# Luka140/paig_reproduction

Hardware: AMD Instinct MI355X
Metric: video-seqs/sec (train step) spring_color B=100 @ 1/2/4/8 MI355X (higher is better)
Workload: dtype fp32; 1 GPU; spring_color PhysicsNet train step (get_batch gather+fwd+loss+bwd+allreduce+RMSprop), B=100/rank, 32x32x3, seq_len 50 (4 in / 6 pred / 40 extrap); global_batch=100, seq_len=50, parallelism=dp1, conv_math=split, split_graph=False, optimizer_in_graph=True, byte_targets=True, dataset_seqs=800

## Files before the change

### paig_reproduction_amd/csrc/conv_split.hip

```cpp
#include "split_common.h"

#ifndef PAIG_FWD_AUXP
#define PAIG_FWD_AUXP 1
#endif

namespace {


constexpr bool sfwd_sla(bool UPS, int PM, int H, int W, int ups_bytes, int lo_bytes) {
  return UPS && PM == 0 && H * W >= 4096 && ups_bytes <= lo_bytes;
}
constexpr int sfwd_lds(int CIN, int H, int W, int KS, bool UPS, int PM, int tpxm, int ntb) {
  const int CC = rup(CIN, 8) / 8, PS = CC % 2 == 0 ? CC + 1 : CC;
  const int NS = ceil_div(KS * KS * CC, 4);
  const int FPT = H * W <= tpxm ? tpxm / (H * W) : 1;
  const int RT = H * W <= tpxm ? H : rows_fit(H, W, tpxm);
  const int TWPX = W + 2 * (KS / 2);
  const int RP = W == 8 ? to_mod16(TWPX * PS, 8) : TWPX * PS;
  const int img = FPT * (RT + KS - 1) * RP * 8, wimg = NS * ntb * 64 * 8;
  const int ups = UPS ? up_window_floats(CIN, FPT, RT, W) * 4 : 0;
  return (img + wimg) * 2 * (PM == 2 ? 1 : 2) + (sfwd_sla(UPS, PM, H, W, ups, img * 2) ? 0 : ups);
}
constexpr int sfwd_vgprs(int CIN, int H, int W, int KS, bool UPS, int tpxm, int ntb) {
  const int CC = rup(CIN, 8) / 8, NS = ceil_div(KS * KS * CC, 4);
  const int FPT = H * W <= tpxm ? tpxm / (H * W) : 1;
  const int RT = H * W <= tpxm ? H : rows_fit(H, W, tpxm);
  const int MW = ceil_div(ceil_div(FPT * RT * W, 16), 4);
  const int NL = UPS ? 1 : ceil_div(FPT * (RT + KS - 1) * (W % 2 == 0 ? W / 2 : W) * CC, 256);
  return MW * ntb * 4 + NL * 30 + ntb * 8 + NS + MW * 8 + 40;
}
#ifndef PAIG_FWD_UPS_TP
#define PAIG_FWD_UPS_TP 256
#endif
#ifndef PAIG_FWD_TP32
#define PAIG_FWD_TP32 256
#endif
constexpr int sfwd_pick(int CIN, int COUT, int H, int W, int KS, bool UPS, int PM) {
  const int base = UPS && H * W < 4096 && PAIG_FWD_UPS_TP < 256   ? PAIG_FWD_UPS_TP
                   : !UPS && H * W == 1024 && PAIG_FWD_TP32 < 256 ? PAIG_FWD_TP32
                                                                  : (W == 8 ? 128 : 256);
  const int NT = ceil_div(COUT, 16);
  for (int pass = UPS && !(PM == 0 && H * W >= 4096) ? 1 : 0; pass < 3; ++pass)
    for (int nb = 1; nb <= NT; ++nb) {
      if (NT % nb != 0 || NT / nb > 4) continue;
      for (int tp = base; tp >= (pass == 1 ? base / 2 : 64); tp /= 2)
        if (sfwd_lds(CIN, H, W, KS, UPS, PM, tp, NT / nb) <= (pass == 0 ? LDS_MAX / 2 : LDS_MAX) &&
            sfwd_vgprs(CIN, H, W, KS, UPS, tp, NT / nb) <= 264 && (pass > 0 || tp >= base / 2))
          return tp * 256 + nb;
    }
  return 0;
}

template <int CIN, int COUT, int H, int W, int KS, bool UPS, int PM>
struct SFwdCfg {
  static constexpr int KK = KS * KS, PADL = KS / 2;
  static constexpr int NIMG = PM == 2 ? 1 : 2;
  static constexpr int CINP = rup(CIN, 8), CC = CINP / 8;
  static constexpr int KC = KK * CC, NS = ceil_div(KC, 4);
  static constexpr int GEO = sfwd_pick(CIN, COUT, H, W, KS, UPS, PM);
  static_assert(GEO > 0, "no forward tile geometry fits the LDS");
  static constexpr int NB = GEO % 256;
  static constexpr int NT = ceil_div(COUT, 16) / NB;
  static constexpr int TPXM = GEO / 256;
  static constexpr int FPT = H * W <= TPXM ? TPXM / (H * W) : 1;
  static constexpr int RT = H * W <= TPXM ? H : rows_fit(H, W, TPXM);
  static constexpr int TPXV = FPT * RT * W;
  static constexpr int NMT = ceil_div(TPXV, 16);
  static constexpr int MW = ceil_div(NMT, 4);
  static constexpr int ROWS = RT + KS - 1;
  static constexpr int TWPX = W + 2 * PADL;
  static constexpr int PS = CC % 2 == 0 ? CC + 1 : CC;
  static constexpr int RP = W == 8 ? to_mod16(TWPX * PS, 8) : TWPX * PS;
  static constexpr int IMG = FPT * ROWS * RP * 8;
  static constexpr int WIMG = NS * NT * 64 * 8;
  static constexpr int SLB = UPS ? up_window_floats(CIN, FPT, RT, W) * 4 : 0;
  static constexpr bool SLA = sfwd_sla(UPS, PM, H, W, SLB, IMG * 2);
  static constexpr int LDS = (IMG + WIMG) * 2 * NIMG + (SLA ? 0 : SLB);
  static constexpr int UPX = W % 2 == 0 ? 2 : 1;
  static constexpr int W2 = W / UPX;
  static constexpr int NI = FPT * ROWS * W2 * CC;
  static constexpr int NL = (NI + 255) / 256;
  static constexpr bool VEC4 = W % 4 == 0;
  static_assert(H % RT == 0, "RT divides H");
  static constexpr int PO = W / 16;
  static constexpr bool POOLOK = !UPS && VEC4 && W % 16 == 0 && PO >= 1 && MW % 2 == 0 && NMT == 4 * MW &&
                                 TPXV % (2 * W) == 0 && RT % 2 == 0;
};

__device__ __forceinline__ float pool4(float a, float b, float c, float d) {
  float m = a;
  if (b > m || b != b) m = b;
  if (c > m || c != c) m = c;
  if (d > m || d != d) m = d;
  return m;
}

__device__ __forceinline__ unsigned char pool_code(float a, float b, float c, float d) {
  float m = a;
  int k = 0;
  if (b > m || b != b) { m = b; k = 1; }
  if (c > m || c != c) { m = c; k = 2; }
  if (d > m || d != d) { m = d; k = 3; }
  return (unsigned char)((a > 0.f ? 1 : 0) | (b > 0.f ? 2 : 0) | (c > 0.f ? 4 : 0) | (d > 0.f ? 8 : 0) | (k << 4));
}

template <int MW, int PO, bool POOL>
__device__ __forceinline__ int fwd_mtile(int wv, int mt) {
  if constexpr (POOL) {
    constexpr int HM = MW / 2;
    const int u = wv * HM + mt % HM;
    return ((u / PO) * 2 + mt / HM) * PO + u % PO;
  } else {
    return wv * MW + mt;
  }
}

template <int CIN, int COUT, int H, int W, int KS, bool DG, bool UPS, int PM, bool POOL = false, bool UPT = false,
          bool PF = false>
__device__ __forceinline__ void conv_fwd_split_body(FView in, FViewW out, FView aux, const float* __restrict__ w,
                                                    const float* __restrict__ bias, int F, int flags, int ntiles, XMax xm,
                                                    const s16x8* __restrict__ wp, PoolOut pout, int bx, int gx) {
  using C = SFwdCfg<CIN, COUT, H, W, KS, UPS, PM>;
  static_assert(!PF || (DG && !UPS && !POOL && !UPT && C::UPX == 2 && H % 2 == 0 && CIN % 8 == 0),
                "pool fold: dgrad staging units of one window's pixel pair");
  static_assert(!UPT || (DG && !UPS && !POOL && C::FPT == 1 && C::RT % 2 == 0 && C::VEC4 && W % 2 == 0),
                "transposed-upsample epilogue: dgrad tiles of whole row pairs");
  constexpr int KK = C::KK, CC = C::CC, KC = C::KC, NS = C::NS, NT = C::NT, MW = C::MW;
  constexpr int RT = C::RT, FPT = C::FPT, ROWS = C::ROWS, PS = C::PS, RP = C::RP;
  constexpr int NI = C::NI, NL = C::NL, PADL = C::PADL, W2 = C::W2;
  constexpr long long PLANE = UPS ? (long long)(H / 2) * (W / 2) : (long long)H * W;
  constexpr long long HW = (long long)H * W;
  extern __shared__ __attribute__((aligned(16))) short lds16[];
  short* Xh = lds16;
  short* Xl = Xh + (C::NIMG == 2 ? C::IMG : 0);
  short* Wh = lds16 + C::NIMG * C::IMG;
  short* Wl = Wh + (C::NIMG == 2 ? C::WIMG : 0);
  const int tid = threadIdx.x, lane = tid & 63, wv = tid >> 6, g = lane >> 4;
  constexpr int NRB = H / RT;
  const int co0 = blockIdx.y * NT * 16;
  float rmax = 0.f;
  __shared__ float smax[4];

  auto wval = [&](int idx, int j) {
    const int ln = idx & 63, snt = idx >> 6, nt = snt % NT, s = snt / NT;
    const int kc = 4 * s + (ln >> 4), co = co0 + nt * 16 + (ln & 15);
    float v = 0.f;
    if (kc < KC && co < COUT) {
      const int tap = kc / CC, ci = (kc % CC) * 8 + j;
      if (ci < CIN) v = DG ? w[(ci * COUT + co) * KK + (KK - 1 - tap)] : w[(co * CIN + ci) * KK + tap];
    }
    return v;
  };
  int ewn[NT];
#pragma unroll
  for (int nt = 0; nt < NT; ++nt) ewn[nt] = 0;
  __shared__ int sew[PM == 0 ? NT * 16 : 1];
  auto zero_halo = [&]() {
    if (PADL > 0) {
      for (int i = tid; i < FPT * ROWS * 2 * PADL * CC; i += 256) {
        const int cc = i % CC, hc = (i / CC) % (2 * PADL), r = i / (CC * 2 * PADL);
        const int xc = hc < PADL ? hc : W + hc;
        const int o = (r * RP + xc * PS + cc) * 8;
        *reinterpret_cast<s16x8*>(Xh + o) = s16x8{0, 0, 0, 0, 0, 0, 0, 0};
        if (PM != 2) *reinterpret_cast<s16x8*>(Xl + o) = s16x8{0, 0, 0, 0, 0, 0, 0, 0};
      }
    }
  };
  zero_halo();
  int pbase[MW];
#pragma unroll
  for (int mt = 0; mt < MW; ++mt) {
    int pix = fwd_mtile<MW, C::PO, POOL>(wv, mt) * 16 + (lane & 15);
    if (pix >= C::TPXV) pix = 0;
    const int fi = pix / (RT * W), rem = pix % (RT * W);
    pbase[mt] = (fi * ROWS + rem / W) * RP + (rem % W) * PS;
  }
  int soff[NS];
#pragma unroll
  for (int s = 0; s < NS; ++s) {
    int kc = 4 * s + g;
    if (kc >= KC) kc = 0;
    const int tap = kc / CC, cc = kc % CC;
    soff[s] = (tap / KS) * RP + (tap % KS) * PS + cc;
  }

  using UP = UpStage<UPS ? CIN : 1, H, W, FPT, RT>;
  float* Sl = reinterpret_cast<float*>(C::SLA ? Xl : lds16 + C::NIMG * (C::IMG + C::WIMG));
  constexpr int UPX = C::UPX;
  auto split_px = [&](int i, const float2* v, float sc, s16x8& h0, s16x8& l0, s16x8& h1, s16x8& l1) {
    const int xp = UPX * (i % W2), r = (i / W2) % ROWS, cc = (i / (W2 * ROWS)) % CC, fi = i / (W2 * ROWS * CC);
    if constexpr (PM == 0) {
      pf32x2 sv[8];
#pragma unroll
      for (int c = 0; c < 8; ++c) sv[c] = pf32x2{v[c].x, v[c].y} * sc;
      u32x4 a0, b0, a1, b1;
#pragma unroll
      for (int k = 0; k < 4; ++k) {
        { const HiLo q_ = split_pk(sv[2 * k].x, sv[2 * k + 1].x); a0[k] = q_.h; b0[k] = q_.l; }
        { const HiLo q_ = split_pk(sv[2 * k].y, sv[2 * k + 1].y); a1[k] = q_.h; b1[k] = q_.l; }
      }
      h0 = __builtin_bit_cast(s16x8, a0);
      l0 = __builtin_bit_cast(s16x8, b0);
      h1 = __builtin_bit_cast(s16x8, a1);
      l1 = __builtin_bit_cast(s16x8, b1);
    }
    return ((fi * ROWS + r) * RP + (xp + PADL) * PS + cc) * 8;
  };
  auto put_px = [&](int i, const float2* v, float sc) {
    const int xp = UPX * (i % W2), r = (i / W2) % ROWS, cc = (i / (W2 * ROWS)) % CC, fi = i / (W2 * ROWS * CC);
    const int o = ((fi * ROWS + r) * RP + (xp + PADL) * PS + cc) * 8;
    s16x8 h0, l0, h1, l1;
    if constexpr (PM == 0) {
      pf32x2 sv[8];
#pragma unroll
      for (int c = 0; c < 8; ++c) sv[c] = pf32x2{v[c].x, v[c].y} * sc;
      u32x4 a0, b0, a1, b1;
#pragma unroll
      for (int k = 0; k < 4; ++k) {
        { const HiLo q_ = split_pk(sv[2 * k].x, sv[2 * k + 1].x); a0[k] = q_.h; b0[k] = q_.l; }
        { const HiLo q_ = split_pk(sv[2 * k].y, sv[2 * k + 1].y); a1[k] = q_.h; b1[k] = q_.l; }
      }
      h0 = __builtin_bit_cast(s16x8, a0);
      l0 = __builtin_bit_cast(s16x8, b0);
      h1 = __builtin_bit_cast(s16x8, a1);
      l1 = __builtin_bit_cast(s16x8, b1);
    } else {
#pragma unroll
      for (int c = 0; c < 8; ++c) {
        short h, lo;
        split<PM>(v[c].x, h, lo, rmax);
        h0[c] = h;
        l0[c] = lo;
        split<PM>(v[c].y, h, lo, rmax);
        h1[c] = h;
        l1[c] = lo;
      }
    }
    *reinterpret_cast<s16x8*>(Xh + o) = h0;
    if (PM != 2) *reinterpret_cast<s16x8*>(Xl + o) = l0;
    if constexpr (UPX == 2) {
      *reinterpret_cast<s16x8*>(Xh + o + PS * 8) = h1;
      if (PM != 2) *reinterpret_cast<s16x8*>(Xl + o + PS * 8) = l1;
    }
  };
  float2 pre[UPS ? 1 : NL][8];
  float dpv[PF ? NL : 1][8];
  uint2 pcv[PF ? NL : 1];
  UP up;
  constexpr bool SCL = PM == 0, DYN = PM == 0 && PAIG_SCALE_MODE < 2;
  float tsc = 1.f, tinv[NT], xrun = 0.f;
#pragma unroll
  for (int nt = 0; nt < NT; ++nt) tinv[nt] = 1.f;
  auto tile_scale = [&]() {
    const float m = fmaxf(fmaxf(smax[0], smax[1]), fmaxf(smax[2], smax[3]));
    xrun = fmaxf(xrun, m);
    const int e = f16_scale_exp(m);
    tsc = __builtin_amdgcn_ldexpf(1.f, e);
#pragma unroll
    for (int nt = 0; nt < NT; ++nt) tinv[nt] = __builtin_amdgcn_ldexpf(1.f, -(e + ewn[nt]));
  };
  auto issue = [&](int t) {
    const int f0 = (t / NRB) * FPT, y0 = (t % NRB) * RT;
    if constexpr (UPS) {
      up.issue(in, F, f0, y0, tid);
    } else {
      const float* fb = in.frame(f0);
#pragma unroll
      for (int l = 0; l < NL; ++l) {
        const int i = tid + l * 256;
        const int xp = UPX * (i % W2), r = (i / W2) % ROWS, cc = (i / (W2 * ROWS)) % CC, fi = i / (W2 * ROWS * CC);
        const int gy = y0 + r - PADL;
        const bool ok = i < NI && f0 + fi < F && gy >= 0 && gy < H;
        const int off = fi * (int)in.fs + cc * 8 * (int)PLANE + gy * W + xp;
        static_assert(8 * PLANE <= 8 * 4096, "paig_zero_planes covers the unit");
        const float* base = ok ? fb + off : paig_zero_planes;
#pragma unroll
        for (int c = 0; c < 8; ++c) {
          const float* q = CIN % 8 == 0 || cc * 8 + c < CIN ? base + c * (int)PLANE : paig_zeros;
          pre[l][c] = UPX == 2 ? *reinterpret_cast<const float2*>(q) : make_float2(*q, 0.f);
        }
        if constexpr (PF) {
          constexpr int HP = H / 2, WP = W / 2;
          const int pw = (gy >> 1) * WP + (xp >> 1);
          const float* pb = ok ? pout.frame(f0) + fi * (int)pout.fs + cc * 8 * (HP * WP) + pw : paig_zero_planes;
#pragma unroll
          for (int c = 0; c < 8; ++c) dpv[l][c] = pb[c * (HP * WP)];
          const unsigned char* cb = ok ? pout.code + (long long)(f0 + fi) * pout.code_fs + ((long long)cc * HP * WP + pw) * 8
                                       : reinterpret_cast<const unsigned char*>(paig_zeros);
          pcv[l] = *reinterpret_cast<const uint2*>(cb);
        }
      }
    }
  };
  auto fold = [&](int t) {
    if constexpr (PF) {
      const int y0 = (t % NRB) * RT;
#pragma unroll
      for (int l = 0; l < NL; ++l) {
        const int i = tid + l * 256;
        const int r = (i / W2) % ROWS;
        const int pr = ((y0 + r - PADL) & 1) * 2;
#pragma unroll
        for (int c = 0; c < 8; ++c) {
          const unsigned b = ((c < 4 ? pcv[l].x : pcv[l].y) >> (8 * (c & 3))) & 255u;
          const int am = (int)(b >> 4) & 3;
          const float vx = pre[l][c].x + (am == pr ? dpv[l][c] : 0.f);
          const float vy = pre[l][c].y + (am == pr + 1 ? dpv[l][c] : 0.f);
          pre[l][c].x = (b >> pr) & 1u ? vx : 0.f;
          pre[l][c].y = (b >> (pr + 1)) & 1u ? vy : 0.f;
        }
      }
    }
  };
  auto commit = [&](int t) {
    if constexpr (DYN) tile_scale();
    if constexpr (UPT) zero_halo();
    if constexpr (UPS) {
      const int f0 = (t / NRB) * FPT, y0 = (t % NRB) * RT;
      up.commit(Sl, tid);
      __syncthreads();
      if constexpr (C::SLA) {
        static_assert(W % 4 == 0 && UPX == 2, "SLA: 4-pixel items");
        constexpr int W4 = W / 4, NIT = ceil_div(NI / 2, 256);
        s16x8 lk[NIT][4];
        int lo_off[NIT][2];
#pragma unroll
        for (int it = 0; it < NIT; ++it) {
          const int i = tid + it * 256;
          lo_off[it][0] = -1;
          if ((NI / 2) % 256 != 0 && i >= NI / 2) break;
          const int q = i % W4, r = (i / W4) % ROWS, cc = (i / (W4 * ROWS)) % CC, fi = i / (W4 * ROWS * CC);
          const int gy = y0 + r - PADL;
          const bool ok = f0 + fi < F && gy >= 0 && gy < H;
          f32x4 o[8];
#pragma unroll
          for (int c = 0; c < 8; ++c)
            o[c] = (ok && cc * 8 + c < CIN) ? UP::row4(Sl, fi, cc * 8 + c, gy, y0, q) : f32x4{0.f, 0.f, 0.f, 0.f};
          const int ia = ((fi * CC + cc) * ROWS + r) * W2 + 2 * q;
#pragma unroll
          for (int u = 0; u < 2; ++u) {
            float2 v[8];
#pragma unroll
            for (int c = 0; c < 8; ++c) v[c] = make_float2(o[c][2 * u], o[c][2 * u + 1]);
            s16x8 h0, h1;
            const int off = split_px(ia + u, v, tsc, h0, lk[it][2 * u], h1, lk[it][2 * u + 1]);
            *reinterpret_cast<s16x8*>(Xh + off) = h0;
            *reinterpret_cast<s16x8*>(Xh + off + PS * 8) = h1;
            lo_off[it][u] = off;
          }
        }
        __syncthreads();
        for (int i = tid; i < FPT * ROWS * 2 * PADL * CC; i += 256) {
          const int cc = i % CC, hc = (i / CC) % (2 * PADL), r = i / (CC * 2 * PADL);
          const int xc = hc < PADL ? hc : W + hc;
          *reinterpret_cast<s16x8*>(Xl + (r * RP + xc * PS + cc) * 8) = s16x8{0, 0, 0, 0, 0, 0, 0, 0};
        }
#pragma unroll
        for (int it = 0; it < NIT; ++it) {
          if (lo_off[it][0] < 0) break;
#pragma unroll
          for (int u = 0; u < 2; ++u) {
            *reinterpret_cast<s16x8*>(Xl + lo_off[it][u]) = lk[it][2 * u];
            *reinterpret_cast<s16x8*>(Xl + lo_off[it][u] + PS * 8) = lk[it][2 * u + 1];
          }
        }
      } else if constexpr (W % 4 == 0) {
        constexpr int W4 = W / 4;
#pragma unroll 1
        for (int i = tid; i < NI / 2; i += 256) {
          const int q = i % W4, r = (i / W4) % ROWS, cc = (i / (W4 * ROWS)) % CC, fi = i / (W4 * ROWS * CC);
          const int gy = y0 + r - PADL;
          const bool ok = f0 + fi < F && gy >= 0 && gy < H;
          f32x4 o[8];
#pragma unroll
          for (int c = 0; c < 8; ++c)
            o[c] = (ok && cc * 8 + c < CIN) ? UP::row4(Sl, fi, cc * 8 + c, gy, y0, q) : f32x4{0.f, 0.f, 0.f, 0.f};
          const int ia = ((fi * CC + cc) * ROWS + r) * W2 + 2 * q;
          float2 v[8];
#pragma unroll
          for (int c = 0; c < 8; ++c) v[c] = make_float2(o[c][0], o[c][1]);
          put_px(ia, v, tsc);
#pragma unroll
          for (int c = 0; c < 8; ++c) v[c] = make_float2(o[c][2], o[c][3]);
          put_px(ia + 1, v, tsc);
        }
      } else {
#pragma unroll 1
        for (int i = tid; i < NI; i += 256) {
          const int xp = UPX * (i % W2), r = (i / W2) % ROWS, cc = (i / (W2 * ROWS)) % CC, fi = i / (W2 * ROWS * CC);
          const int gy = y0 + r - PADL;
          const bool ok = f0 + fi < F && gy >= 0 && gy < H;
          float2 v[8];
#pragma unroll
          for (int c = 0; c < 8; ++c)
            v[c] = (ok && cc * 8 + c < CIN)
                       ? make_float2(UP::px1(Sl, fi, cc * 8 + c, gy, y0, xp),
                                     UPX == 2 ? UP::px1(Sl, fi, cc * 8 + c, gy, y0, xp + 1) : 0.f)
                       : make_float2(0.f, 0.f);
          put_px(i, v, tsc);
        }
      }
    } else {
#pragma unroll
      for (int l = 0; l < NL; ++l) {
        const int i = tid + l * 256;
        if (NI % 256 != 0 && i >= NI) break;
        put_px(i, pre[l], tsc);
      }
    }
  };

  auto tile_max = [&]() {
    float m = 0.f;
    if constexpr (UPS) {
      m = up.amax();
    } else {
#pragma unroll
      for (int l = 0; l < NL; ++l)
#pragma unroll
        for (int c = 0; c < 8; ++c) m = amax2(m, pre[l][c].x, pre[l][c].y);
    }
    m = wave_max_u(m);
    if (lane == 0) smax[wv] = m;
  };

  int lt = UPT ? 0 : bx;
  const int lstep = UPT ? 1 : gx;
  auto tile_of = [&](int l) {
    if constexpr (UPT) {
      const int f = bx + (l / NRB) * gx;
      return f < F ? f * NRB + l % NRB : ntiles;
    } else {
      return l < ntiles ? xcd_tile(l, ntiles) : ntiles;
    }
  };
  issue(tile_of(lt));
  if (PM == 0 && wp != nullptr) {
    constexpr int NTT = NT * C::NB, WLO = NS * NTT * 64, HDR = NTT * 16 * 4 / 16;
    const int* hdr = reinterpret_cast<const int*>(wp);
#pragma unroll
    for (int nt = 0; nt < NT; ++nt) ewn[nt] = hdr[co0 + nt * 16 + (lane & 15)];
    const s16x8* img = wp + HDR;
    for (int idx = tid; idx < NS * NT * 64; idx += 256) {
      const int s = idx / (NT * 64), r = idx - s * (NT * 64);
      const int src = (s * NTT + blockIdx.y * NT) * 64 + r;
      *reinterpret_cast<s16x8*>(Wh + idx * 8) = img[src];
      *reinterpret_cast<s16x8*>(Wl + idx * 8) = img[WLO + src];
    }
  } else {
    if constexpr (PM == 0) {
      for (int i = tid; i < NT * 16; i += 256) sew[i] = 0;
      __syncthreads();
      float pm[NT];
#pragma unroll
      for (int nt = 0; nt < NT; ++nt) pm[nt] = 0.f;
      for (int idx = tid; idx < NS * NT * 64; idx += 256) {
        const int nt = (idx >> 6) % NT;
#pragma unroll
        for (int j = 0; j < 8; ++j) pm[nt] = fmaxf(pm[nt], fabsf(wval(idx, j)));
      }
#pragma unroll
      for (int nt = 0; nt < NT; ++nt) atomicMax(&sew[nt * 16 + (tid & 15)], __builtin_bit_cast(int, pm[nt]));
      __syncthreads();
      for (int i = tid; i < NT * 16; i += 256) sew[i] = f16_scale_exp_v(__builtin_bit_cast(float, sew[i]));
      __syncthreads();
#pragma unroll
      for (int nt = 0; nt < NT; ++nt) ewn[nt] = sew[nt * 16 + (lane & 15)];
    }
    for (int idx = tid; idx < NS * NT * 64; idx += 256) {
      const int cl = ((idx >> 6) % NT) * 16 + (idx & 15);
      const int e = PM == 0 ? sew[cl] : 0;
      s16x8 vh, vl;
#pragma unroll
      for (int j = 0; j < 8; ++j) {
        short h, l;
        split<PM>(__builtin_amdgcn_ldexpf(wval(idx, j), e), h, l, rmax);
        vh[j] = h;
        vl[j] = l;
      }
      *reinterpret_cast<s16x8*>(Wh + idx * 8) = vh;
      if (PM != 2) *reinterpret_cast<s16x8*>(Wl + idx * 8) = vl;
    }
  }
  if constexpr (!DYN) {
#pragma unroll
    for (int nt = 0; nt < NT; ++nt) tinv[nt] = __builtin_amdgcn_ldexpf(1.f, -ewn[nt]);
  }
  float bvs[NT];
#pragma unroll
  for (int nt = 0; nt < NT; ++nt) {
    const int co = co0 + nt * 16 + (lane & 15);
    bvs[nt] = *(bias && co < COUT ? bias + co : paig_zeros);
    asm volatile("" ::"v"(bvs[nt]));
  }
  constexpr int WS2 = W / 2, NCL = NT * 16, NUI = UPT ? ceil_div(NCL * WS2, 256) : 1;
  float car0[NUI], car1[NUI];
  float auxu[UPT ? NUI : 1][UPT ? RT / 2 + 1 : 1];
  auto upt_aux = [&](int tile) {
    if constexpr (UPT) {
      if (flags & 2) {
        const int f = tile / NRB, kA = (tile % NRB) * (RT / 2);
#pragma unroll
        for (int u = 0; u < NUI; ++u) {
          const int item = tid + u * 256;
          const int cl = item / WS2, j = item % WS2;
          const bool ok = (NCL * WS2) % 256 == 0 || item < NCL * WS2;
#pragma unroll
          for (int i = 0; i <= RT / 2; ++i) {
            const int k = kA - 1 + i;
            const float* ap = aux.frame(f) + (long long)(co0 + cl) * ((H / 2) * WS2) + (long long)k * WS2 + j;
            auxu[u][i] = *(ok && k >= 0 && k < H / 2 ? ap : paig_zeros);
          }
        }
      }
    }
  };
  auto upt_epilogue = [&](int tile, f32x4 (&a)[MW][NT]) {
    constexpr int HS = H / 2, KR = RT / 2 + 2;
    static_assert(!UPT || RT * NCL * W * 4 <= C::NIMG * C::IMG * 2, "the dX tile fits the image's LDS");
    const int f = tile / NRB, band = tile % NRB, kA = band * (RT / 2);
    __syncthreads();
    float* RB = reinterpret_cast<float*>(lds16);
#pragma unroll
    for (int nt = 0; nt < NT; ++nt) {
      const int cl = nt * 16 + (lane & 15);
#pragma unroll
      for (int mt = 0; mt < MW; ++mt) {
        const int pix = fwd_mtile<MW, C::PO, false>(wv, mt) * 16 + (lane >> 4) * 4;
        if (pix >= C::TPXV) continue;
        f32x4 v = a[mt][nt];
        if constexpr (SCL) v *= tinv[nt];
#pragma unroll
        for (int r = 0; r < 4; ++r) v[r] += bvs[nt];
        *reinterpret_cast<f32x4*>(RB + ((pix / W) * NCL + cl) * W + pix % W) = v;
      }
    }
    __syncthreads();
#pragma unroll
    for (int u = 0; u < NUI; ++u) {
      const int item = tid + u * 256;
      if ((NCL * WS2) % 256 != 0 && item >= NCL * WS2) break;
      const int cl = item / WS2, j = item % WS2, co = co0 + cl;
      float P[KR];
      P[0] = band == 0 ? 0.f : car0[u];
      P[1] = band == 0 ? 0.f : car1[u];
#pragma unroll
      for (int i = 2; i < KR; ++i) P[i] = 0.f;
      const float wxa = j >= 1 ? 0.25f : 0.f, wxb = j == 0 ? 1.f : 0.75f;
      const float wxc = j == WS2 - 1 ? 1.f : 0.75f, wxd = j <= WS2 - 2 ? 0.25f : 0.f;
#pragma unroll
      for (int r = 0; r < RT; ++r) {
        const float* rp = RB + (r * NCL + cl) * W + 2 * j;
        const float2 m2 = *reinterpret_cast<const float2*>(rp);
        float hs = 0.f;
        if (wxa != 0.f) hs = fmaf(wxa, rp[-1], hs);
        hs = fmaf(wxb, m2.x, hs);
        hs = fmaf(wxc, m2.y, hs);
        if (wxd != 0.f) hs = fmaf(wxd, rp[2], hs);
        const int m = kA + r / 2;
        if (r % 2 == 0) {
          if (m >= 1) P[r / 2] = fmaf(0.25f, hs, P[r / 2]);
          P[r / 2 + 1] = fmaf(m == 0 ? 1.f : 0.75f, hs, P[r / 2 + 1]);
        } else {
          P[r / 2 + 1] = fmaf(m == HS - 1 ? 1.f : 0.75f, hs, P[r / 2 + 1]);
          if (m + 1 <= HS - 1) P[r / 2 + 2] = fmaf(0.25f, hs, P[r / 2 + 2]);
        }
      }
      const bool last = band == NRB - 1;
      const long long po = (long long)co * (HS * WS2) + j;
#pragma unroll
      for (int i = 0; i <= RT / 2; ++i) {
        const int k = kA - 1 + i;
        if (k < 0 || (i == RT / 2 && !last)) continue;
        float v = P[i];
        if (flags & 2) v = auxu[u][i] > 0.f ? v : 0.f;
        out.frame(f)[po + k * WS2] = v;
      }
      car0[u] = P[RT / 2];
      car1[u] = P[RT / 2 + 1];
    }
  };
  for (;; lt += lstep) {
    const int tile = tile_of(lt);
    if (tile >= ntiles) break;
    const int f0 = (tile / NRB) * FPT, y0 = (tile % NRB) * RT;
    fold(tile);
    if constexpr (DYN) tile_max();
    __syncthreads();
    commit(tile);
    __syncthreads();
    constexpr bool AUXP = PAIG_FWD_AUXP && DG && C::VEC4 && !POOL && !UPT && MW * NT <= 8;
    f32x4 auxv[AUXP ? MW : 1][AUXP ? NT : 1];
    if constexpr (AUXP) {
      if (flags & 2) {
#pragma unroll
        for (int nt = 0; nt < NT; ++nt) {
          const int co = co0 + nt * 16 + (lane & 15);
#pragma unroll
          for (int mt = 0; mt < MW; ++mt) {
            const int pix = fwd_mtile<MW, C::PO, POOL>(wv, mt) * 16 + (lane >> 4) * 4;
            const int fi = pix / (RT * W), rem = pix % (RT * W);
            const int f = f0 + fi;
            const bool ok = co < COUT && pix < C::TPXV && f < F;
            const float* ap = ok ? aux.frame(f) + co * HW + (long long)(y0 + rem / W) * W + rem % W : paig_zero_planes;
            auxv[mt][nt] = *reinterpret_cast<const f32x4*>(ap);
          }
        }
      }
    }
    upt_aux(tile);
    issue(tile_of(lt + lstep));
    f32x4 acc[MW][NT];
#pragma unroll
    for (int mt = 0; mt < MW; ++mt)
#pragma unroll
      for (int nt = 0; nt < NT; ++nt) acc[mt][nt] = f32x4{0.f, 0.f, 0.f, 0.f};
#pragma unroll
    for (int s = 0; s < NS; ++s) {
      s16x8 bh[NT], bl[NT];
#pragma unroll
      for (int nt = 0; nt < NT; ++nt) {
        const int o = ((s * NT + nt) * 64 + lane) * 8;
        bh[nt] = *reinterpret_cast<const s16x8*>(Wh + o);
        bl[nt] = PM != 2 ? *reinterpret_cast<const s16x8*>(Wl + o) : bh[nt];
      }
#pragma unroll
      for (int mt = 0; mt < MW; ++mt) {
        const int o = (pbase[mt] + soff[s]) * 8;
        const s16x8 ah = *reinterpret_cast<const s16x8*>(Xh + o);
        const s16x8 al = PM != 2 ? *reinterpret_cast<const s16x8*>(Xl + o) : ah;
#pragma unroll
        for (int nt = 0; nt < NT; ++nt) acc[mt][nt] = mma3<PM>(ah, al, bh[nt], bl[nt], acc[mt][nt]);
      }
    }
    if constexpr (UPT) {
      upt_epilogue(tile, acc);
      continue;
    }
#pragma unroll
    for (int nt = 0; nt < NT; ++nt) {
      const int co = co0 + nt * 16 + (lane & 15);
      if (co >= COUT) continue;
      const float bv = bvs[nt];
      f32x4 vv[MW];
#pragma unroll
      for (int mt = 0; mt < MW; ++mt) {
        const int pix = fwd_mtile<MW, C::PO, POOL>(wv, mt) * 16 + (lane >> 4) * 4;
        if constexpr (C::VEC4) {
          if (pix >= C::TPXV) continue;
          const int fi = pix / (RT * W), rem = pix % (RT * W);
          const int y = y0 + rem / W, x = rem % W, f = f0 + fi;
          if (f >= F) continue;
          float* op = out.frame(f) + co * HW + (long long)y * W + x;
          f32x4 v = acc[mt][nt];
          if constexpr (SCL) v *= tinv[nt];
#pragma unroll
          for (int r = 0; r < 4; ++r) v[r] += bv;
          if (flags & 1) {
#pragma unroll
            for (int r = 0; r < 4; ++r) v[r] = v[r] < 0.f ? 0.f : v[r];
          }
          if (flags & 4) v += *reinterpret_cast<const f32x4*>(op);
          if (flags & 2) {
            f32x4 m;
            if constexpr (AUXP) m = auxv[mt][nt];
            else m = *reinterpret_cast<const f32x4*>(aux.frame(f) + co * HW + (long long)y * W + x);
#pragma unroll
            for (int r = 0; r < 4; ++r) v[r] = m[r] > 0.f ? v[r] : 0.f;
          }
          *reinterpret_cast<f32x4*>(op) = v;
          if constexpr (POOL) vv[mt] = v;
        } else {
#pragma unroll
          for (int r = 0; r < 4; ++r) {
            const int pr = pix + r;
            if (pr >= C::TPXV) break;
            const int fi = pr / (RT * W), rem = pr % (RT * W);
            const int y = y0 + rem / W, x = rem % W, f = f0 + fi;
            if (f >= F) continue;
            float* op = out.frame(f) + co * HW + (long long)y * W + x;
            float v = (SCL ? acc[mt][nt][r] * tinv[nt] : acc[mt][nt][r]) + bv;
            if (flags & 1) v = v < 0.f ? 0.f : v;
            if (flags & 4) v += *op;
            if (flags & 2) v = aux.frame(f)[co * HW + (long long)y * W + x] > 0.f ? v : 0.f;
            *op = v;
          }
        }
      }
// ... 732 lines not shown
__global__ void __launch_bounds__(256, 2)
conv_fwd_wprep_k(FView in, FViewW out, FView aux, const float* __restrict__ w, const float* __restrict__ bias, int F,
                 int flags, int ntiles, XMax xm, PoolOut pout, WPrepJobs jobs, int nwp) {
  if ((int)blockIdx.x < nwp) {
    conv_wprep_body(jobs, blockIdx.x);
    return;
  }
  conv_fwd_split_body<CIN, COUT, H, W, KS, false, false, PM>(in, out, aux, w, bias, F, flags, ntiles, xm, nullptr, pout,
                                                            (int)blockIdx.x - nwp, (int)gridDim.x - nwp);
}

WPrepJobs g_wpend{};
int g_wpend_blocks = 0;
int wprep_build(WPrepJobs& jobs, int n, const float* const* w, const int* cin, const int* cout, const int* ks,
                const int* dg, void* const* out, int* blocks_out) {
  jobs = WPrepJobs{};
  jobs.n = n;
  int blocks = 0;
  for (int q = 0; q < n; ++q) {
    PAIG_REQUIRE(w[q] && out[q] && cin[q] > 0 && cout[q] > 0 && ks[q] > 0, "conv_wprep: job %d", q);
    PAIG_REQUIRE(((uintptr_t)out[q] & 15) == 0, "conv_wprep: job %d output not 16-byte aligned", q);
    jobs.j[q] = WPrepJob{w[q], static_cast<s16x8*>(out[q]), cin[q], cout[q], ks[q], dg[q]};
    jobs.blk0[q] = blocks;
    if (dg[q] == 2) {
      blocks += (cin[q] + 31) / 32 * ((cout[q] + 31) / 32);
      continue;
    }
    const int NS = (ks[q] * ks[q] * ((cin[q] + 7) / 8) + 3) / 4;
    blocks += (cout[q] + 15) / 16 * ((NS + WPREP_S - 1) / WPREP_S);
  }
  jobs.blk0[n] = blocks;
  *blocks_out = blocks;
  return 0;
}
int wprep_flush(hipStream_t st) {
  if (!g_wpend_blocks) return 0;
  const int nb = g_wpend_blocks;
  g_wpend_blocks = 0;
  hipLaunchKernelGGL(conv_wprep_k, dim3(nb), dim3(WPREP_T), 0, st, g_wpend);
  PAIG_CHECK_LAUNCH();
  return 0;
}

static int g_fwd_block_cap = 0;
static XMax g_prezero{};

template <int CIN, int COUT, int H, int W, int KS, bool DG, bool UPS, int PM, bool UPT = false, bool PF = false>
static int sfwd_launch(FView in, FViewW out, FView aux, const float* w, const float* b, int F, int flags,
                       hipStream_t st, XMax xm, const void* wp, PoolOut pout) {
  using C = SFwdCfg<CIN, COUT, H, W, KS, UPS, PM>;
  constexpr int LDS = C::LDS;
  static_assert(C::SLB == (UPS ? UpStage<CIN, H, W, C::FPT, C::RT>::SL * 4 : 0), "upsample window bytes");
  const int ntiles = cdiv(F, C::FPT) * (H / C::RT);
  constexpr bool POOLABLE = C::POOLOK && !DG;
  auto k = PF ? conv_fwd_split_k<CIN, COUT, H, W, KS, DG, UPS, PM, false, false, PF>
         : UPT ? conv_fwd_split_k<CIN, COUT, H, W, KS, DG, UPS, PM, false, UPT>
              : (POOLABLE && (flags & 64)) ? conv_fwd_split_k<CIN, COUT, H, W, KS, DG, UPS, PM, POOLABLE>
                                           : conv_fwd_split_k<CIN, COUT, H, W, KS, DG, UPS, PM, false>;
  static int resident[2] = {0, 0};
  const int kv = (POOLABLE && (flags & 64)) ? 1 : 0;
  if (!resident[kv]) {
    if (LDS > 64 * 1024) (void)hipFuncSetAttribute((const void*)k, hipFuncAttributeMaxDynamicSharedMemorySize, LDS);
    resident[kv] = persistent_grid((const void*)k, LDS);
  }
  static const int bpc = [] {
    const char* e = getenv("PAIG_FWD_BPC");
    return e ? atoi(e) : 0;
  }();
  int res = resident[kv];
  if (bpc > 0 && res > bpc * 256) res = bpc * 256;
  int nb = res / C::NB;
  if (nb > (UPT ? F : ntiles)) nb = UPT ? F : ntiles;
  if (g_fwd_block_cap > 0 && nb > g_fwd_block_cap) nb = g_fwd_block_cap;
  if (nb < 1) nb = 1;
  if (PM != 0 || DG) xm.p = nullptr;
  PAIG_REQUIRE(!xm.p || nb <= xm.n, "conv split fwd: %d blocks need more than %d xmax slots", nb, xm.n);
  if (xm.p && g_prezero.z) {
    xm.z = g_prezero.z;
    xm.zn = g_prezero.zn;
    g_prezero = XMax{};
  }
  if (PF) PAIG_REQUIRE(pout.p && pout.code, "conv split dgrad: the pool fold needs the pooled gradient and codes");
  else if (flags & 64) PAIG_REQUIRE(C::POOLOK && pout.p, "conv split fwd: no fused pool for Cin=%d Cout=%d H=%d", CIN, COUT, H);
  if constexpr (CIN == 3 && PM == 0 && !DG && !UPS && !UPT && !PF && C::NB == 1) {
    if (g_wpend_blocks && !(flags & 64)) {
      auto km = conv_fwd_wprep_k<CIN, COUT, H, W, KS, PM>;
      static bool attr = false;
      if (!attr && LDS > 64 * 1024) (void)hipFuncSetAttribute((const void*)km, hipFuncAttributeMaxDynamicSharedMemorySize, LDS);
      attr = true;
      const int nwp = g_wpend_blocks;
      g_wpend_blocks = 0;
      hipLaunchKernelGGL(km, dim3(nwp + nb), dim3(256), LDS, st, in, out, aux, w, b, F, flags, ntiles, xm, pout, g_wpend,
                         nwp);
      PAIG_CHECK_LAUNCH();
      return 0;
    }
  }
  if (int rc = wprep_flush(st)) return rc;
  hipLaunchKernelGGL(k, dim3(nb, C::NB), dim3(256), LDS, st, in, out, aux, w, b, F, flags, ntiles, xm,
                     PM == 0 ? static_cast<const s16x8*>(wp) : nullptr, pout);
  PAIG_CHECK_LAUNCH();
  return 0;
}

template <int CIN, int COUT, int H, int W, int KS, bool UPS, int PM, bool PF = false>
static int swg_launch(FView x, FView dy, float* slab, int nblk_max, int* nblk_out, int F, hipStream_t st, XMax xm,
                      PoolOut pin = PoolOut{nullptr, 0, nullptr, 0}) {
  using C = SWgCfg<CIN, COUT, H, W, KS, UPS, PM>;
  constexpr int STG = C::STG + (UPS && !C::SLA ? UpStage<C::CINB, H, W, C::FPT, C::RT>::SL * 4 : 0);
  constexpr int LDS = STG > C::RED ? STG : C::RED;
  const int ntiles = cdiv(F, C::FPT) * (H / C::RT);
  auto k = conv_wgrad_split_k<CIN, COUT, H, W, KS, UPS, PM, PF>;
  if constexpr (PF) PAIG_REQUIRE(pin.p && pin.code, "conv split wgrad: the pool fold needs the pooled gradient and codes");
  static int resident = 0;
  if (!resident) {
    if (LDS > 64 * 1024) (void)hipFuncSetAttribute((const void*)k, hipFuncAttributeMaxDynamicSharedMemorySize, LDS);
    resident = persistent_grid((const void*)k, LDS);
  }
  int nb = ntiles < nblk_max ? ntiles : nblk_max;
  if (nb > resident / (C::NSI * C::NSO)) nb = resident / (C::NSI * C::NSO);
  if (nb < 1) nb = 1;
  *nblk_out = nb;
  PAIG_REQUIRE(!xm.p || (xm.n % 4 == 0 && (reinterpret_cast<uintptr_t>(xm.p) & 15) == 0),
               "conv split wgrad: xmax needs 16-byte alignment and a multiple of 4 slots (%d)", xm.n);
  hipLaunchKernelGGL(k, dim3(nb, C::NSI, C::NSO), dim3(256), LDS, st, x, dy, slab, F, ntiles, xm, pin);
  PAIG_CHECK_LAUNCH();
  return 0;
}

#define PAIG_SPLIT_FWD(X)                                                                                 \
  X(3, 8, 32, 3) X(8, 8, 32, 3) X(8, 16, 16, 3) X(16, 16, 16, 3) X(16, 32, 8, 3) X(32, 32, 8, 3)         \
  X(32, 16, 16, 3) X(16, 16, 32, 3) X(24, 8, 32, 3) X(8, 2, 32, 1) X(16, 8, 16, 3) X(8, 24, 32, 3)       \
  X(2, 8, 32, 1) X(32, 16, 8, 3) X(16, 32, 16, 3)                                                         \
  PAIG_SPLIT_FWD_3BP(X) PAIG_SPLIT_FWD_UNET(X)
#define PAIG_SPLIT_WG(X)                                                                                  \
  X(3, 8, 32, 3) X(8, 8, 32, 3) X(8, 16, 16, 3) X(16, 16, 16, 3) X(16, 32, 8, 3) X(32, 32, 8, 3)         \
  X(32, 16, 16, 3) X(16, 16, 32, 3) X(24, 8, 32, 3) X(8, 2, 32, 1)                                        \
  PAIG_SPLIT_WG_3BP(X) PAIG_SPLIT_WG_UNET(X)
#define PAIG_SPLIT_UP(X)                                                                                  \
  X(32, 16, 16, 3) X(16, 16, 32, 3) X(32, 16, 18, 3) X(16, 16, 36, 3) X(128, 32, 16, 3) X(64, 32, 32, 3) \
  X(32, 32, 64, 3)
#define PAIG_SPLIT_PF(X) X(32, 32, 32, 3) PAIG_SPLIT_PF_C6(X)
#ifndef PAIG_PF_C6
#define PAIG_PF_C6 0
#endif
#if PAIG_PF_C6
#define PAIG_SPLIT_PF_C6(X) X(64, 64, 16, 3)
#else
#define PAIG_SPLIT_PF_C6(X)
#endif
#define PAIG_SPLIT_UPT(X) X(32, 128, 16, 3) X(32, 64, 32, 3) X(32, 32, 64, 3)
#define PAIG_SPLIT_FWD_3BP(X)                                                                             \
  X(3, 8, 36, 3) X(8, 8, 36, 3) X(8, 16, 18, 3) X(16, 16, 18, 3) X(16, 32, 9, 3) X(32, 32, 9, 3)         \
  X(32, 16, 18, 3) X(16, 16, 36, 3) X(24, 8, 36, 3) X(8, 3, 36, 1) X(16, 8, 18, 3) X(32, 16, 9, 3)       \
  X(16, 32, 18, 3) X(8, 24, 36, 3) X(3, 8, 36, 1)
#define PAIG_SPLIT_FWD_UNET(X)                                                                            \
  X(3, 16, 64, 3) X(16, 16, 64, 3) X(16, 32, 32, 3) X(32, 32, 32, 3) X(32, 64, 16, 3) X(64, 64, 16, 3)   \
  X(64, 128, 8, 3) X(128, 128, 8, 3) X(96, 64, 16, 3) X(64, 32, 32, 3) X(48, 16, 64, 3) X(16, 2, 64, 1)   \
  X(32, 16, 32, 3) X(64, 32, 16, 3) X(128, 64, 8, 3) X(32, 128, 16, 3) X(64, 96, 16, 3) X(32, 64, 32, 3)  \
  X(32, 32, 64, 3) X(16, 48, 64, 3) X(2, 16, 64, 1)
#define PAIG_SPLIT_WG_UNET(X)                                                                             \
  X(3, 16, 64, 3) X(16, 16, 64, 3) X(16, 32, 32, 3) X(32, 32, 32, 3) X(32, 64, 16, 3) X(64, 64, 16, 3)   \
  X(64, 128, 8, 3) X(128, 128, 8, 3) X(96, 64, 16, 3) X(64, 32, 32, 3) X(48, 16, 64, 3) X(16, 2, 64, 1)
#define PAIG_SPLIT_WG_3BP(X)                                                                              \
  X(3, 8, 36, 3) X(8, 8, 36, 3) X(8, 16, 18, 3) X(16, 16, 18, 3) X(16, 32, 9, 3) X(32, 32, 9, 3)         \
  X(32, 16, 18, 3) X(16, 16, 36, 3) X(24, 8, 36, 3) X(8, 3, 36, 1)
// ... 194 lines not shown
```

Baseline: 102,800 video-seqs/s.

## Use buffer-resource loads with hoisted addresses and early weight prefetch in split conv forward

Replaces pointer-select global loads in the split-conv forward/dgrad staging (input, pooled gradient, codes, aux masks) with raw buffer loads that rely on out-of-range offsets returning zero. Per-thread address offsets are hoisted out of the tile loop for some shapes, and bias plus the first few weight-image chunks are prefetched into registers before the halo zeroing. A per-shape form table keeps the old path for some layers, and a host check confirms frame strides fit 32-bit byte offsets. The aim is to cut address arithmetic and branchy zero-pointer selects and to overlap the weight fetch with setup, at the cost of extra registers.

After: 104,200 video-seqs/s, median of 6. 1.4% higher.

```diff
diff --git a/paig_reproduction_amd/csrc/conv_split.hip b/paig_reproduction_amd/csrc/conv_split.hip
--- a/paig_reproduction_amd/csrc/conv_split.hip
+++ b/paig_reproduction_amd/csrc/conv_split.hip
@@ -50,6 +50,15 @@
     }
   return 0;
 }
+
+constexpr int sfwd_form(int CIN, int COUT, int H, int PM, bool POOL) {
+  if (CIN == 16 && COUT == 48 && H == 64) return 0;
+  if (CIN == 64 && COUT == 96 && H == 16 && POOL) return 0;
+  if (PM == 2 && CIN == 3 && COUT == 16 && H == 64 && POOL) return 0;
+  if (PM == 2 && COUT == 32 && H == 32 && (CIN == 16 || CIN == 32) && !POOL) return 0;
+  return PM == 2 ? 1 : 2;
+}
+constexpr int SFWD_WEARLY = 6;
 
 template <int CIN, int COUT, int H, int W, int KS, bool UPS, int PM>
 struct SFwdCfg {
@@ -155,6 +164,29 @@
 #pragma unroll
   for (int nt = 0; nt < NT; ++nt) ewn[nt] = 0;
   __shared__ int sew[PM == 0 ? NT * 16 : 1];
+  constexpr int NTT = NT * C::NB, WLO = NS * NTT * 64, WSL = NS * NT * 64, WHDR = NTT * 16 * 4;
+  constexpr int FORM = sfwd_form(CIN, COUT, H, PM, POOL);
+  constexpr bool HOIST = FORM == 2;
+  constexpr int WNE = PM == 0 && FORM > 0 ? (ceil_div(WSL, 256) < SFWD_WEARLY ? ceil_div(WSL, 256) : SFWD_WEARLY) : 0;
+  float bvs[NT];
+  s16x8 wph[WNE > 0 ? WNE : 1], wpl[WNE > 0 ? WNE : 1];
+  if constexpr (FORM > 0) {
+    const brsrc rb = buf_rsrc(bias, bias ? COUT * 4 : 0);
+#pragma unroll
+    for (int nt = 0; nt < NT; ++nt) bvs[nt] = buf_ld1(rb, (co0 + nt * 16 + (lane & 15)) * 4, 0);
+    if constexpr (WNE > 0) {
+      const brsrc rw = buf_rsrc(wp, wp ? WHDR + 2 * WLO * 16 : 0);
+#pragma unroll
+      for (int nt = 0; nt < NT; ++nt) ewn[nt] = __builtin_bit_cast(int, buf_ld1(rw, (co0 + (lane & 15)) * 4, nt * 64));
+#pragma unroll
+      for (int k = 0; k < WNE; ++k) {
+        const int idx = tid + k * 256, s = idx / (NT * 64), r = idx - s * (NT * 64);
+        const int vo = (WSL % 256 == 0 || idx < WSL) ? ((s * NTT + (int)blockIdx.y * NT) * 64 + r) * 16 : BUF_OOR;
+        wph[k] = __builtin_bit_cast(s16x8, buf_ld4(rw, vo, WHDR));
+        wpl[k] = __builtin_bit_cast(s16x8, buf_ld4(rw, vo, WHDR + WLO * 16));
+      }
+    }
+  }
   auto zero_halo = [&]() {
     if (PADL > 0) {
       for (int i = tid; i < FPT * ROWS * 2 * PADL * CC; i += 256) {
@@ -166,7 +198,7 @@
       }
     }
   };
-  zero_halo();
+  if constexpr (FORM == 0) zero_halo();
   int pbase[MW];
 #pragma unroll
   for (int mt = 0; mt < MW; ++mt) {
@@ -259,11 +291,47 @@
 #pragma unroll
     for (int nt = 0; nt < NT; ++nt) tinv[nt] = __builtin_amdgcn_ldexpf(1.f, -(e + ewn[nt]));
   };
+  auto row_ok = [&](int gy) { return (unsigned)gy < (unsigned)H; };
+  auto s_unit = [&](int i, int& vo, int& row) {
+    const int xp = UPX * (i % W2), r = (i / W2) % ROWS, cc = (i / (W2 * ROWS)) % CC, fi = i / (W2 * ROWS * CC);
+    row = i < NI ? r - PADL : -(1 << 20);
+    vo = ((FPT > 1 ? fi * (int)in.fs : 0) + cc * 8 * (int)PLANE + (r - PADL) * W + xp) * 4;
+    if (NRB == 1 && !row_ok(row)) vo = BUF_OOR;
+  };
+  constexpr int NLH = HOIST && !UPS ? NL : 1;
+  int svo[NLH], srow[NLH];
+  if constexpr (HOIST && !UPS) {
+#pragma unroll
+    for (int l = 0; l < NL; ++l) s_unit(tid + l * 256, svo[l], srow[l]);
+  }
+  auto s_get = [&](int l, int& vo, int& row) {
+    if constexpr (HOIST) {
+      vo = svo[l];
+      row = srow[l];
+    } else {
+      s_unit(opaque(tid) + l * 256, vo, row);
+    }
+  };
+  auto pf_unit = [&](int i, int& po, int& co) {
+    constexpr int HP = H / 2, WP = W / 2;
+    const int xp = UPX * (i % W2), cc = (i / (W2 * ROWS)) % CC, fi = i / (W2 * ROWS * CC);
+    po = ((FPT > 1 ? fi * (int)pout.fs : 0) + cc * 8 * (HP * WP) + (xp >> 1)) * 4;
+    co = (FPT > 1 ? fi * (int)pout.code_fs : 0) + (cc * (HP * WP) + (xp >> 1)) * 8;
+  };
+  constexpr int NUH = HOIST && UPS ? UP::NLS : 1;
+  int uvo[NUH], urow[NUH];
+  if constexpr (HOIST && UPS) {
+#pragma unroll
+    for (int l = 0; l < UP::NLS; ++l) UP::unit(tid + l * 256, (int)in.fs, uvo[l], urow[l]);
+  }
+  auto tile_nf = [&](int f0) {
+    const int n = F - f0;
+    return n < FPT ? n : FPT;
+  };
+  static_assert(FORM > 0 || (!UPS && !UPT && !PF), "the address-select form covers the plain forward / dgrad only");
   auto issue = [&](int t) {
-    const int f0 = (t / NRB) * FPT, y0 = (t % NRB) * RT;
-    if constexpr (UPS) {
-      up.issue(in, F, f0, y0, tid);
-    } else {
+    const int f0 = (t / NRB) * FPT, y0 = (t % NRB) * RT, nf = tile_nf(f0);
+    if constexpr (FORM == 0) {
       const float* fb = in.frame(f0);
 #pragma unroll
       for (int l = 0; l < NL; ++l) {
@@ -279,15 +347,54 @@
           const float* q = CIN % 8 == 0 || cc * 8 + c < CIN ? base + c * (int)PLANE : paig_zeros;
           pre[l][c] = UPX == 2 ? *reinterpret_cast<const float2*>(q) : make_float2(*q, 0.f);
         }
+      }
+      return;
+    }
+    const brsrc rin = tile_rsrc(in.frame(f0), in.fs, nf, CIN * (int)PLANE);
+    if constexpr (UPS) {
+      if constexpr (HOIST) {
+        up.issue(rin, y0, uvo, urow);
+      } else {
+        int uo[UP::NLS], ur[UP::NLS];
+#pragma unroll
+        for (int l = 0; l < UP::NLS; ++l) UP::unit(opaque(tid) + l * 256, (int)in.fs, uo[l], ur[l]);
+        up.issue(rin, y0, uo, ur);
+      }
+    } else {
+      brsrc rp, rc;
+      if constexpr (PF) {
+        rp = tile_rsrc(pout.frame(f0), pout.fs, nf, CIN * (H / 2) * (W / 2));
+        rc = tile_rsrc(pout.code + (long long)f0 * pout.code_fs, pout.code_fs, nf, CC * (H / 2) * (W / 2) * 8, 1);
+      }
+#pragma unroll
+      for (int l = 0; l < NL; ++l) {
+        int vo0, row;
+        s_get(l, vo0, row);
+        const int vo = NRB == 1 ? vo0 : (row_ok(y0 + row) ? vo0 + y0 * W * 4 : BUF_OOR);
+#pragma unroll
+        for (int c = 0; c < 8; ++c) {
+          int voc = vo;
+          if constexpr (CIN % 8 != 0) {
+            if (CC == 1 && c >= CIN) {
+              pre[l][c] = make_float2(0.f, 0.f);
+              continue;
+            }
+            if (c >= CIN % 8 && ((tid + l * 256) / (W2 * ROWS)) % CC == CC - 1) voc = BUF_OOR;
+          }
+          pre[l][c] = UPX == 2 ? buf_ld2(rin, voc, c * (int)PLANE * 4) : make_float2(buf_ld1(rin, voc, c * (int)PLANE * 4), 0.f);
+        }
         if constexpr (PF) {
           constexpr int HP = H / 2, WP = W / 2;
-          const int pw = (gy >> 1) * WP + (xp >> 1);
-          const float* pb = ok ? pout.frame(f0) + fi * (int)pout.fs + cc * 8 * (HP * WP) + pw : paig_zero_planes;
-#pragma unroll
-          for (int c = 0; c < 8; ++c) dpv[l][c] = pb[c * (HP * WP)];
-          const unsigned char* cb = ok ? pout.code + (long long)(f0 + fi) * pout.code_fs + ((long long)cc * HP * WP + pw) * 8
-                                       : reinterpret_cast<const unsigned char*>(paig_zeros);
-          pcv[l] = *reinterpret_cast<const uint2*>(cb);
+          const int gy = y0 + row;
+          const bool ok = NRB == 1 ? vo != BUF_OOR : row_ok(gy);
+          int po, co;
+          pf_unit(opaque(tid) + l * 256, po, co);
+          const int wr = (gy >> 1) * WP;
+          const int vp = ok ? po + wr * 4 : BUF_OOR;
+#pragma unroll
+          for (int c = 0; c < 8; ++c) dpv[l][c] = buf_ld1(rp, vp, c * (HP * WP) * 4);
+          const u32x2 cv = __builtin_amdgcn_raw_buffer_load_b64(rc, ok ? co + wr * 8 : BUF_OOR, 0, 0);
+          pcv[l] = make_uint2(cv.x, cv.y);
         }
       }
     }
@@ -435,13 +542,23 @@
     }
   };
   issue(tile_of(lt));
+  if constexpr (FORM > 0) zero_halo();
   if (PM == 0 && wp != nullptr) {
-    constexpr int NTT = NT * C::NB, WLO = NS * NTT * 64, HDR = NTT * 16 * 4 / 16;
-    const int* hdr = reinterpret_cast<const int*>(wp);
-#pragma unroll
-    for (int nt = 0; nt < NT; ++nt) ewn[nt] = hdr[co0 + nt * 16 + (lane & 15)];
+    constexpr int HDR = WHDR / 16;
+    if constexpr (WNE == 0) {
+      const int* hdr = reinterpret_cast<const int*>(wp);
+#pragma unroll
+      for (int nt = 0; nt < NT; ++nt) ewn[nt] = hdr[co0 + nt * 16 + (lane & 15)];
+    }
+#pragma unroll
+    for (int k = 0; k < WNE; ++k) {
+      const int idx = tid + k * 256;
+      if (WSL % 256 != 0 && idx >= WSL) break;
+      *reinterpret_cast<s16x8*>(Wh + idx * 8) = wph[k];
+      *reinterpret_cast<s16x8*>(Wl + idx * 8) = wpl[k];
+    }
     const s16x8* img = wp + HDR;
-    for (int idx = tid; idx < NS * NT * 64; idx += 256) {
+    for (int idx = tid + WNE * 256; idx < WSL; idx += 256) {
       const int s = idx / (NT * 64), r = idx - s * (NT * 64);
       const int src = (s * NTT + blockIdx.y * NT) * 64 + r;
       *reinterpret_cast<s16x8*>(Wh + idx * 8) = img[src];
@@ -486,30 +603,40 @@
 #pragma unroll
     for (int nt = 0; nt < NT; ++nt) tinv[nt] = __builtin_amdgcn_ldexpf(1.f, -ewn[nt]);
   }
-  float bvs[NT];
 #pragma unroll
   for (int nt = 0; nt < NT; ++nt) {
-    const int co = co0 + nt * 16 + (lane & 15);
-    bvs[nt] = *(bias && co < COUT ? bias + co : paig_zeros);
+    if constexpr (FORM == 0) {
+      const int co = co0 + nt * 16 + (lane & 15);
+      bvs[nt] = *(bias && co < COUT ? bias + co : paig_zeros);
+    }
     asm volatile("" ::"v"(bvs[nt]));
   }
   constexpr int WS2 = W / 2, NCL = NT * 16, NUI = UPT ? ceil_div(NCL * WS2, 256) : 1;
   float car0[NUI], car1[NUI];
   float auxu[UPT ? NUI : 1][UPT ? RT / 2 + 1 : 1];
+  auto upt_unit = [&](int item) {
+    const int cl = item / WS2, j = item % WS2;
+    return (NCL * WS2) % 256 == 0 || item < NCL * WS2 ? ((co0 + cl) * ((H / 2) * WS2) + j) * 4 : BUF_OOR;
+  };
+  int avu[UPT && HOIST ? NUI : 1];
+  if constexpr (UPT && HOIST) {
+#pragma unroll
+    for (int u = 0; u < NUI; ++u) avu[u] = upt_unit(tid + u * 256);
+  }
   auto upt_aux = [&](int tile) {
     if constexpr (UPT) {
       if (flags & 2) {
         const int f = tile / NRB, kA = (tile % NRB) * (RT / 2);
+        const brsrc ra = tile_rsrc(aux.frame(f), aux.fs, 1, COUT * (H / 2) * WS2);
 #pragma unroll
         for (int u = 0; u < NUI; ++u) {
-          const int item = tid + u * 256;
-          const int cl = item / WS2, j = item % WS2;
-          const bool ok = (NCL * WS2) % 256 == 0 || item < NCL * WS2;
+          int vo;
+          if constexpr (HOIST) vo = avu[u];
+          else vo = upt_unit(opaque(tid) + u * 256);
 #pragma unroll
           for (int i = 0; i <= RT / 2; ++i) {
             const int k = kA - 1 + i;
-            const float* ap = aux.frame(f) + (long long)(co0 + cl) * ((H / 2) * WS2) + (long long)k * WS2 + j;
-            auxu[u][i] = *(ok && k >= 0 && k < H / 2 ? ap : paig_zeros);
+            auxu[u][i] = buf_ld1(ra, (unsigned)k < (unsigned)(H / 2) ? vo + k * WS2 * 4 : BUF_OOR, 0);
           }
         }
       }
@@ -580,6 +707,17 @@
       car1[u] = P[RT / 2 + 1];
     }
   };
+  constexpr bool AUXP = PAIG_FWD_AUXP && DG && C::VEC4 && !POOL && !UPT && MW * NT <= 8;
+  auto a_unit = [&](int wave, int ln, int mt) {
+    const int pix = fwd_mtile<MW, C::PO, POOL>(wave, mt) * 16 + (ln >> 4) * 4;
+    const int fi = pix / (RT * W), rem = pix % (RT * W);
+    return pix < C::TPXV ? ((FPT > 1 ? fi * (int)aux.fs : 0) + (co0 + (ln & 15)) * (int)HW + rem) * 4 : BUF_OOR;
+  };
+  int avo[AUXP && HOIST ? MW : 1];
+  if constexpr (AUXP && HOIST) {
+#pragma unroll
+    for (int mt = 0; mt < MW; ++mt) avo[mt] = a_unit(wv, lane, mt);
+  }
   for (;; lt += lstep) {
     const int tile = tile_of(lt);
     if (tile >= ntiles) break;
@@ -589,9 +727,8 @@
     __syncthreads();
     commit(tile);
     __syncthreads();
-    constexpr bool AUXP = PAIG_FWD_AUXP && DG && C::VEC4 && !POOL && !UPT && MW * NT <= 8;
     f32x4 auxv[AUXP ? MW : 1][AUXP ? NT : 1];
-    if constexpr (AUXP) {
+    if constexpr (AUXP && FORM == 0) {
       if (flags & 2) {
 #pragma unroll
         for (int nt = 0; nt < NT; ++nt) {
@@ -604,6 +741,21 @@
             const bool ok = co < COUT && pix < C::TPXV && f < F;
             const float* ap = ok ? aux.frame(f) + co * HW + (long long)(y0 + rem / W) * W + rem % W : paig_zero_planes;
             auxv[mt][nt] = *reinterpret_cast<const f32x4*>(ap);
+          }
+        }
+      }
+    } else if constexpr (AUXP) {
+      if (flags & 2) {
+        const brsrc ra = tile_rsrc(aux.frame(f0), aux.fs, tile_nf(f0), COUT * (int)HW);
+#pragma unroll
+        for (int nt = 0; nt < NT; ++nt) {
+          const bool cok = co0 + nt * 16 + (lane & 15) < COUT;
+#pragma unroll
+          for (int mt = 0; mt < MW; ++mt) {
+            int vo;
+            if constexpr (HOIST) vo = avo[mt];
+            else vo = a_unit(opaque(wv), opaque(lane), mt);
+            auxv[mt][nt] = buf_ld4(ra, cok ? vo : BUF_OOR, (nt * 16 * (int)HW + y0 * W) * 4);
           }
         }
       }
@@ -1502,6 +1654,15 @@
   }
   if (PF) PAIG_REQUIRE(pout.p && pout.code, "conv split dgrad: the pool fold needs the pooled gradient and codes");
   else if (flags & 64) PAIG_REQUIRE(C::POOLOK && pout.p, "conv split fwd: no fused pool for Cin=%d Cout=%d H=%d", CIN, COUT, H);
+  if constexpr (C::FPT > 1) {
+    constexpr long long SPAN = (1ll << 31) / (4 * (C::FPT - 1)) - 8 * 4096;
+    constexpr long long INF = (long long)CIN * (UPS ? (H / 2) * (W / 2) : H * W), HP2 = (H / 2) * (W / 2);
+    const bool mask = DG && (flags & 2) && aux.p;
+    PAIG_REQUIRE(in.fs >= INF && in.fs < SPAN && (!mask || (aux.fs >= (long long)COUT * H * W && aux.fs < SPAN)) &&
+                     (!PF || (pout.fs >= CIN * HP2 && pout.fs < SPAN && pout.code_fs >= C::CC * HP2 * 8 &&
+                              pout.code_fs < 4 * SPAN)),
+                 "conv split fwd: a frame stride is below the frame's size or does not fit the tile's 32-bit byte offsets");
+  }
   if constexpr (CIN == 3 && PM == 0 && !DG && !UPS && !UPT && !PF && C::NB == 1) {
     if (g_wpend_blocks && !(flags & 64)) {
       auto km = conv_fwd_wprep_k<CIN, COUT, H, W, KS, PM>;
```
